# asmekal/ubdvss

Measured on AMD Instinct MI355X. Metric: images/sec (512x512) fwd+CCL, higher is better.
Workload: dtype f32; 1 GPU; configs[1]: batch=32 512x512x3 fp32 forward + CCL postprocess per GPU (stripe-textured rectangle images, random-init weights); batch_per_gpu=32, parallelism=replicas x1, no collective

## Files before the change

ubdvss_amd/csrc/api.hip:

```cpp
#include <stdarg.h>
#include <stddef.h>
#include <stdlib.h>
#include <string.h>
#include <thread>
#include "common.h"

static thread_local char g_err[512] = "";

void ubd_set_error(const char *fmt, ...)
{
    va_list ap;
    va_start(ap, fmt);
    vsnprintf(g_err, sizeof(g_err), fmt, ap);
    va_end(ap);
}

extern "C" const char *ubd_last_error(void) { return g_err; }
extern "C" int ubd_abi_version(void) { return UBD_ABI_VERSION; }
#ifndef UBD_BUILD_ID
#define UBD_BUILD_ID "unknown"
#endif
extern "C" int ubd_host_memcpy_mt(void *dst, const void *src, size_t n, int threads)
{
    if (threads < 1) threads = 1;
// ... 18 lines not shown
    memcpy(dst, src, done_to);
    for (int t = 0; t < started; ++t) th[t].join();
    return 0;
}
extern "C" const char *ubd_build_id(void) { return UBD_BUILD_ID; }

#ifdef UBD_STAMPS
static struct { const char *kernel; ubd_stamp_buf buf; int sel0, sel1; } g_stamps[] = {
    {"stem23"}, {"stem123"}, {"wino"}, {"wino6"}, {"sep123_16"}, {"dilconv16s"}, {"sepb16"}, {"sep_bwd"}, {"dil_wgrad16"}, {"postprocess"}, {"loss"},
};
extern "C" int ubd_debug_set_stamps(const char *kernel, void *buf, size_t capacity_words, int sel0, int sel1)
{
    for (auto &e : g_stamps)
        if (kernel && strcmp(kernel, e.kernel) == 0) {
            e.buf = {(unsigned long long *)buf, buf ? capacity_words : 0};
            e.sel0 = sel0; e.sel1 = sel1;
            return 0;
        }
    UBD_REQUIRE(false, "ubd_debug_set_stamps: no kernel family named %s", kernel ? kernel : "(null)");
}
ubd_stamp_buf ubd_stamps_for(const char *kernel, int sel0, int sel1)
{
    for (const auto &e : g_stamps)
        if (strcmp(kernel, e.kernel) == 0) return e.sel0 == sel0 && e.sel1 == sel1 ? e.buf : ubd_stamp_buf{nullptr, 0};
    return {nullptr, 0};
}
#endif

static const char ANY[] = "", NUMBER[] = "#";
struct env_switch { const char *name; size_t field; const char *value; int set; };
#define SW(name, field, value, set) {name, offsetof(ubd_handle, field), value, set}
static const env_switch ENV_SWITCHES[] = {
    SW("UBD_DILCONV", use_wino, "direct", 0), SW("UBD_DILCONV", wino_x6, "direct", 0), SW("UBD_DILCONV", wino_x6, "wino32", 0),
    SW("UBD_WINO6_LAYOUT", wino6_natural, "natural", 1),
    SW("UBD_STEM", fuse_stem, "fused", UBD_STEM_FUSED23), SW("UBD_STEM", fuse_force, "fused", 1),
    SW("UBD_STEM", fuse_stem, "fused123", UBD_STEM_FUSED123), SW("UBD_STEM", fuse_force, "fused123", 1),
    SW("UBD_STEM", fuse_stem, "unfused", UBD_STEM_SEPARATE),
    SW("UBD_TEST_NUM_CUS", num_cus, NUMBER, 0),
    SW("UBD_DILBWD", split_dilbwd, "split", 1), SW("UBD_DILBWD", no_pair_dilbwd, "pair8", 1),
    SW("UBD_SEPBWD", split_sepbwd32, "split", 1),
    SW("UBD_STEM16", split_stem16, "split", 1), SW("UBD_STEM16", split_stem16, "fused12", 2),
    SW("UBD_PP_GLOBAL", pp_global, ANY, 1), SW("UBD_PP_SPLIT", pp_split, ANY, 1), SW("UBD_PP_POISON", pp_poison, ANY, 1),
    SW("UBD_PP_SERIAL_TAIL", pp_serial_tail, ANY, 1), SW("UBD_PP_THREADS_512", pp_threads_512, ANY, 1),
    SW("UBD_HEADBWD", split_headbwd, "split", 1),
    SW("UBD_SEPB16_X", sepb_x_regs, "regs", 1),
    SW("UBD_REDUCE", chain_reduce, "batched", 0),
    SW("UBD_LOSS", loss_chain, "chain", 1),
    SW("UBD_DILCONV16", direct_dil16, "direct", 1),
};
#undef SW

extern "C" int ubd_create(const ubd_config *cfg, ubd_handle **out)
{
    UBD_REQUIRE(cfg && out, "ubd_create: null argument");
    UBD_REQUIRE(cfg->c_in == 1 || cfg->c_in == 3, "ubd_create: c_in must be 1 (grey) or 3, got %d", cfg->c_in);
    UBD_REQUIRE(cfg->n_classes >= 0 && cfg->n_classes <= UBD_MAX_CLASSES, "ubd_create: n_classes %d out of range [0,%d]", cfg->n_classes, UBD_MAX_CLASSES);
    UBD_REQUIRE(cfg->dtype == UBD_F32 || cfg->dtype == UBD_BF16 || cfg->dtype == UBD_F16, "ubd_create: bad dtype %d", cfg->dtype);
    int ndev = 0;
    hipError_t e = hipGetDeviceCount(&ndev);
    UBD_REQUIRE(e == hipSuccess && ndev > 0, "ubd_create: no HIP device visible (%s); this library has no CPU fallback", hipGetErrorString(e));
    int dev = 0;
    UBD_CHECK_HIP(hipGetDevice(&dev));
    hipDeviceProp_t prop;
    UBD_CHECK_HIP(hipGetDeviceProperties(&prop, dev));
    UBD_REQUIRE(strncmp(prop.gcnArchName, "gfx950", 6) == 0, "ubd_create: device arch %s is not gfx950; this library is built for MI355X only", prop.gcnArchName);

// ... 45 lines not shown
```

ubdvss_amd/csrc/common.h:

```cpp
#pragma once
#include <hip/hip_runtime.h>
#include <stdint.h>
#include <stdio.h>
#include <string.h>
#include <type_traits>
#include "../../include/ubd.h"
#include "stem_plan.h"
#include "stamps.h"

#define UBD_C 24
#define UBD_NUM_DIL 6

struct ubd_comm;
struct ubd_handle {
    ubd_config cfg;
    ubd_comm *comm;
    int k_out;
    size_t off_sep_dw[3], off_sep_pw[3], off_sep_b[3];
    size_t off_dil_k[UBD_NUM_DIL], off_dil_b[UBD_NUM_DIL];
    size_t off_head_k, off_head_b;
    size_t n_params;
    int num_cus;
    int pp_lds_attr_set;
    int stem_cold_tail;
    int fuse_force;
    int split_headbwd;
    int no_pair_dilbwd;
    int split_dilbwd;
    int split_stem16;
    int pp_global, pp_split, pp_poison, pp_serial_tail, pp_threads_512;
    int sepb_x_regs;
    int split_sepbwd32;
    int chain_reduce;
    int direct_dil16;
    int fuse_stem;
    int use_wino;
    int loss_chain;
    int wino_x6;
    int wino6_natural;
};

static const int UBD_DILATIONS[UBD_NUM_DIL] = {1, 2, 4, 8, 16, 1};

#if defined(__HIPCC__)
__device__ __forceinline__ int ubd_xcd_tile(int L, int total)
{
    return (total & 7) == 0 ? (L & 7) * (total >> 3) + (L >> 3) : L;
}
#endif

#if defined(__HIPCC__)
__device__ __forceinline__ void ubd_glds16_at(const void *gsrc, unsigned lds_dst)
{
    unsigned keep;
    asm volatile("s_mov_b32 %0, m0\n\ts_mov_b32 m0, %2\n\ts_nop 0\n\tglobal_load_lds_dwordx4 %1, off\n\ts_mov_b32 m0, %0"
                 : "=&s"(keep) : "v"(gsrc), "s"(lds_dst) : "memory");
}
__device__ __forceinline__ void ubd_glds16_sbase(const void *base_uniform, unsigned voff, unsigned lds_dst)
{
    unsigned keep;
    asm volatile("s_mov_b32 %0, m0\n\ts_mov_b32 m0, %3\n\ts_nop 0\n\tglobal_load_lds_dwordx4 %1, %2\n\ts_mov_b32 m0, %0"
                 : "=&s"(keep) : "v"(voff), "s"(base_uniform), "s"(lds_dst) : "memory");
}
__device__ __forceinline__ void ubd_blds16(__amdgpu_buffer_rsrc_t rsrc, unsigned voff, unsigned lds_dst)
{
    unsigned keep;
    asm volatile("s_mov_b32 %0, m0\n\ts_mov_b32 m0, %3\n\ts_nop 0\n\tbuffer_load_dwordx4 %1, %2, 0 offen lds\n\ts_mov_b32 m0, %0"
                 : "=&s"(keep) : "v"(voff), "s"(rsrc), "s"(lds_dst) : "memory");
}
__device__ __forceinline__ void ubd_blds4(__amdgpu_buffer_rsrc_t rsrc, unsigned voff, unsigned lds_dst)
{
// ... 64 lines not shown
                          hipGetErrorString(_e));                                        \
            return 1;                                                                    \
        }                                                                                \
    } while (0)

#define UBD_REQUIRE(cond, ...)                                                           \
    do {                                                                                 \
        if (!(cond)) {                                                                   \
            ubd_set_error(__VA_ARGS__);                                                  \
            return 2;                                                                    \
        }                                                                                \
    } while (0)

static inline size_t ubd_align_up(size_t v, size_t a) { return (v + a - 1) / a * a; }

static inline bool ubd_pixels_by_lds_dma(bool f32_in, float sub, float div, int H, int W, int c_in, size_t limit, const void *x)
{
    return f32_in && sub == 0.f && div == 1.f && (size_t)H * W * c_in * 4 < limit && ((uintptr_t)x & 15) == 0;
}
static inline bool ubd_head_in_epilogue(const ubd_handle *h) { return h->k_out == 1 && h->off_head_b == h->off_head_k + UBD_C; }
template <int V> using ubd_int = std::integral_constant<int, V>;
template <typename F> static inline void ubd_dispatch_bool(bool b, F f) { if (b) f(std::true_type{}); else f(std::false_type{}); }
template <typename F> static inline void ubd_dispatch_input(int c_in, bool u8, F f)
{
    if (c_in == 1) { if (u8) f(ubd_int<1>{}, ubd_int<1>{}); else f(ubd_int<1>{}, ubd_int<0>{}); }
    else { if (u8) f(ubd_int<3>{}, ubd_int<1>{}); else f(ubd_int<3>{}, ubd_int<0>{}); }
}

#define UBD_DIL_FRAG_FLOATS (9 * 6 * 2 * 64)
#define UBD_SEP_FRAG_FLOATS (6 * 2 * 64)
#define UBD_SEP_DW_FLOATS (9 * 6 * 64)
#define UBD_WINO_FRAG_FLOATS (16 * 6 * 64 * 2)
#define UBD_FWD_DIRECT_FLOATS (3 * (UBD_SEP_FRAG_FLOATS + UBD_SEP_DW_FLOATS) + UBD_NUM_DIL * UBD_DIL_FRAG_FLOATS)
#define UBD_WINO6_FRAG_U32 (16 * 2 * 3 * 64 * 4)
#define UBD_FWD_WINO6_OFF (UBD_FWD_DIRECT_FLOATS + UBD_NUM_DIL * UBD_WINO_FRAG_FLOATS)
#define UBD_FWD_FRAG_FLOATS (UBD_FWD_WINO6_OFF + UBD_NUM_DIL * UBD_WINO6_FRAG_U32)

struct ubd_fwd_layout {
    size_t off_tickets;
    size_t off_wfrag;
    size_t off_a1, off_a2;
    size_t off_b[2];
    size_t off_acts[7];
    size_t total;
};

bool ubd_comm_fused(const ubd_handle *h);
bool ubd_comm_global_loss(const ubd_handle *h);
int ubd_comm_rank(const ubd_handle *h);
enum { UBD_RED_F64 = 0, UBD_RED_I32 = 1, UBD_RED_U32 = 2 };
int ubd_comm_allreduce_raw(ubd_handle *h, void *buf, size_t count, int kind, hipStream_t st);
int ubd_comm_allgather_u32(ubd_handle *h, const unsigned *send_one, unsigned *recv_world, hipStream_t st);
extern "C" int ubd_comm_world(const ubd_handle *h);
int ubd_comm_begin_tail(ubd_handle *h, float *grads, hipStream_t st);
int ubd_comm_finish(ubd_handle *h, float *grads, hipStream_t st);
void ubd_fwd_layout_compute(const ubd_handle *h, int n, int H, int W, int training, ubd_fwd_layout *L);
struct pp_lds_args;
int ubd_forward_impl(ubd_handle *h, const float *params, const void *images, int in_dtype, int preprocessing,
                     int n, int H, int W, float *logits, char *ws, const ubd_fwd_layout &L, hipStream_t st, bool inference = false,
                     const pp_lds_args *pp_job = nullptr);
int ubd_pp_fill_job(ubd_handle *hd, const float *logits, int n, int map_h, int map_w, float logit_threshold, int scale, float min_area,
                    int32_t *binary_map, int32_t *quads, int32_t *classes, int32_t *counts, int cap, void *workspace,
                    size_t workspace_bytes, int threads, pp_lds_args *job);
void ubd_launch_dilconv(const ubd_handle *h, int epi, const float *frag, const float *aux, int dilation,
                        const float *in, float *out, int n, int H4, int W4, hipStream_t st);
int ubd_grid_for(long waves_needed, int num_cus, int waves_per_block, int blocks_per_cu);
int ubd_loss_impl(const float *logits, int k_out, const int32_t *y_true, long npix, float *loss, float *dlogits,
                  char *ws, hipStream_t st, ubd_handle *h = nullptr, bool prezeroed = false);
size_t ubd_loss_zero_bytes(void);
// ... 23 lines not shown
```

ubdvss_amd/csrc/forward.hip:

```cpp
#include "common.h"

typedef float f32x4 __attribute__((ext_vector_type(4)));
typedef float f32x2 __attribute__((ext_vector_type(2)));
typedef unsigned int u32x4 __attribute__((ext_vector_type(4)));
typedef unsigned int u32x2 __attribute__((ext_vector_type(2)));

#include "pack.h"
__global__ void pack_weights_kernel(const float *__restrict__ params, float *__restrict__ wfrag, pack_args a)
{
    pack_weights_body(params, wfrag, a, (int)(blockIdx.x * blockDim.x + threadIdx.x), (int)(gridDim.x * blockDim.x));
}

__device__ __forceinline__ void store_tile_relu(float *__restrict__ y, size_t row_base_elems, int x0, int ow,
                                                int lane, f32x4 acc0, f32x4 acc1, float b0, float b1)
{
    const int co = lane & 15, q = lane >> 4;
    const unsigned long long rp = (unsigned long long)(y + (row_base_elems + (size_t)x0) * UBD_C);
    const unsigned rlo = (unsigned)__builtin_amdgcn_readfirstlane((int)(unsigned)rp);
    const unsigned rhi = (unsigned)__builtin_amdgcn_readfirstlane((int)(unsigned)(rp >> 32));
    float *rowp = (float *)(((unsigned long long)rhi << 32) | rlo);
    int npx = ow - x0 < 16 ? ow - x0 : 16;
    npx = npx < 0 ? 0 : npx;
    const unsigned bytes = (unsigned)__builtin_amdgcn_readfirstlane(npx * UBD_C * 4);
    __amdgpu_buffer_rsrc_t rs = __builtin_amdgcn_make_buffer_rsrc((void *)rowp, 0, (int)bytes, 0x00020000);
// ... 537 lines not shown
void ubd_launch_pack_direct(const ubd_handle *h, const float *params, float *wfrag, hipStream_t st)
{
    pack_args pa;
    for (int s = 0; s < 3; ++s) { pa.off_sep_dw[s] = h->off_sep_dw[s]; pa.off_sep_pw[s] = h->off_sep_pw[s]; }
    for (int k = 0; k < UBD_NUM_DIL; ++k) pa.off_dil_k[k] = h->off_dil_k[k];
    pa.c_in = h->cfg.c_in;
    hipLaunchKernelGGL(pack_weights_kernel, dim3(64), dim3(256), 0, st, params, wfrag, pa);
}

static void launch_pack(const ubd_handle *h, const float *params, float *wfrag, hipStream_t st)
{
    ubd_launch_pack_direct(h, params, wfrag, st);
    if (h->use_wino) ubd_launch_pack_wino(h, params, wfrag + UBD_FWD_DIRECT_FLOATS, 0, st);
    if (h->wino_x6) ubd_launch_pack_wino6(h, params, (unsigned *)(wfrag + UBD_FWD_WINO6_OFF), st);
}

void ubd_launch_dilconv(const ubd_handle *h, int epi, const float *frag, const float *aux, int dilation,
                        const float *in, float *out, int n, int H4, int W4, hipStream_t st)
{
    const unsigned in_bytes = (unsigned)((size_t)n * H4 * W4 * UBD_C * 4);
    const long tiles = (long)n * H4 * ((W4 + 15) / 16);
    int grid = ubd_grid_for(tiles, h->num_cus, 4, 2);
    grid = (grid + 7) / 8 * 8;
    if (epi == 0)
        hipLaunchKernelGGL(dilconv_f32_kernel<0>, dim3(grid), dim3(256), 0, st, in, out, frag, aux, n, H4, W4, dilation, in_bytes);
    else
        hipLaunchKernelGGL(dilconv_f32_kernel<1>, dim3(grid), dim3(256), 0, st, in, out, frag, aux, n, H4, W4, dilation, in_bytes);
}

static void launch_dil(const ubd_handle *h, const float *params, const float *wfrag, int k, const float *in, float *out,
                       int n, int H4, int W4, hipStream_t st, int lay_in = 1, int lay_out = 1)
{
    if (h->wino_x6) {
        ubd_launch_dilconv_wino6(h, 0, (const unsigned *)(wfrag + UBD_FWD_WINO6_OFF) + (size_t)k * UBD_WINO6_FRAG_U32, params + h->off_dil_b[k],
                                 UBD_DILATIONS[k], in, out, n, H4, W4, st, nullptr, lay_in, lay_out);
        return;
    }
    if (h->use_wino) {
        ubd_launch_dilconv_wino(h, 0, wfrag + UBD_FWD_DIRECT_FLOATS + (size_t)k * UBD_WINO_FRAG_FLOATS, params + h->off_dil_b[k], UBD_F32,
                                UBD_DILATIONS[k], in, out, n, H4, W4, st);
        return;
    }
    const int per_sep = UBD_SEP_FRAG_FLOATS + UBD_SEP_DW_FLOATS;
    const float *dfrag = wfrag + 3 * per_sep;
    ubd_launch_dilconv(h, 0, dfrag + (size_t)k * UBD_DIL_FRAG_FLOATS, params + h->off_dil_b[k], UBD_DILATIONS[k], in, out, n, H4, W4, st);
}

extern "C" int ubd_pack_weights(ubd_handle *h, const float *params, void *workspace, size_t workspace_bytes, void *stream)
{
    UBD_REQUIRE(h && params && workspace, "ubd_pack_weights: null argument");
    if (h->cfg.dtype != UBD_F32) return ubd_pack16_workspace(h, params, (char *)workspace, workspace_bytes, (hipStream_t)stream);
    ubd_fwd_layout L;
    ubd_fwd_layout_compute(h, 1, 4, 4, 0, &L);
    UBD_REQUIRE(workspace_bytes >= L.off_a1, "ubd_pack_weights: workspace too small");
    launch_pack(h, params, (float *)((char *)workspace + L.off_wfrag), (hipStream_t)stream);
    UBD_CHECK_HIP(hipMemsetAsync((char *)workspace + L.off_tickets, 0, 256, (hipStream_t)stream));
    UBD_CHECK_HIP(hipGetLastError());
    return 0;
}

extern "C" int ubd_dilated_layer(ubd_handle *h, const float *params, int layer, const void *in, void *out, int n,
                                 int map_h, int map_w, const void *workspace, void *stream)
{
    UBD_REQUIRE(h && params && in && out && workspace, "ubd_dilated_layer: null argument");
    UBD_REQUIRE(layer >= 0 && layer < UBD_NUM_DIL, "ubd_dilated_layer: layer %d out of range", layer);
    UBD_REQUIRE(h->cfg.dtype == UBD_F32, "ubd_dilated_layer: only UBD_F32 in this build");
    UBD_REQUIRE((size_t)n * map_h * map_w * UBD_C * 4 <= (1ull << 30), "ubd_dilated_layer: tensor too large (activation bytes must not exceed 2^30)");
// ... 76 lines not shown
    static_assert(UBD_STEM_STRIP_ROWS == s23_cfg::TH3, "stem_plan.h counts the strips the stem kernels walk");
    const ubd_stem_plan plan = plan_stem_of(h, n, H, W, inference, pp_job ? pp_job->n : -1);
    UBD_REQUIRE(!plan.job_without_strips, "ubd_forward: a postprocess job needs the fused stem kernel (internal error)");
    const bool one_kernel = plan.form == UBD_STEM_FORM_STRIPS || plan.form == UBD_STEM_FORM_COLD;
    static const int phase_lay[UBD_NUM_DIL + 1] = {2, 4, 1, 1, 1, 2, 1};
    const bool phase_major = h->wino_x6 && !h->wino6_natural && one_kernel;
    const int a3_l2p = phase_major ? 1 : 0;
    int *ticket = (int *)(ws + L.off_tickets);
    if (plan.form == UBD_STEM_FORM_COLD)
        launch_stem123<true>(h, params, images, u8, cur, sf0, sf1, sf2, n, H, W, sc, sh, plan.strips * (W4 <= 16 ? 1 : 1 + (W4 - 16 + 14) / 15),
                             ticket, nullptr, a3_l2p, 0, st);
    else if (plan.form == UBD_STEM_FORM_STRIPS)
        launch_stem123<false>(h, params, images, u8, cur, sf0, sf1, sf2, n, H, W, sc, sh, plan.strips, ticket, pp_job, a3_l2p, plan.tail_rows, st);
    else if (h->cfg.c_in == 1)
        launch_sep<1, 2>(h, images, u8, a1, sf0, params + h->off_sep_b[0], n, H, W, H2, W2, pad_s2, sc, sh, st);
    else
        launch_sep<3, 2>(h, images, u8, a1, sf0, params + h->off_sep_b[0], n, H, W, H2, W2, pad_s2, sc, sh, st);
    if (plan.form == UBD_STEM_FORM_L1_STEM23) {
        const int grid = plan.strips < h->num_cus ? (int)plan.strips : h->num_cus;
        ubd_dispatch_bool(pad_s2 != 0, [&](auto pad) {
            hipLaunchKernelGGL(stem23_kernel<decltype(pad)::value>, dim3(grid), dim3(s23_cfg::NT), 0, st, a1, cur, sf1, params + h->off_sep_b[1], sf2,
                               params + h->off_sep_b[2], n, H2, W2, H4, W4, pad_s2 UBD_STAMP_ARG("stem23"));
        });
    } else if (plan.form == UBD_STEM_FORM_SEPARATE) {
        launch_sep<UBD_C, 1>(h, a1, 0, a2, sf1, params + h->off_sep_b[1], n, H2, W2, H2, W2, 1, 0.f, 1.f, st);
        launch_sep<UBD_C, 2>(h, a2, 0, cur, sf2, params + h->off_sep_b[2], n, H2, W2, H4, W4, pad_s2, 0.f, 1.f, st);
    }

    const bool fuse_head = inference && h->use_wino && ubd_head_in_epilogue(h);
    for (int k = 0; k < UBD_NUM_DIL; ++k) {
        float *nxt = (float *)(ws + L.off_acts[k + 1]);
        if (fuse_head && k == UBD_NUM_DIL - 1) {
            if (h->wino_x6)
                ubd_launch_dilconv_wino6(h, 2, (const unsigned *)(wfrag + UBD_FWD_WINO6_OFF) + (size_t)k * UBD_WINO6_FRAG_U32, params + h->off_dil_b[k],
                                         UBD_DILATIONS[k], cur, logits, n, H4, W4, st, params + h->off_head_k, phase_major ? phase_lay[k] : 1, 1);
            else
                ubd_launch_dilconv_wino(h, 2, wfrag + UBD_FWD_DIRECT_FLOATS + (size_t)k * UBD_WINO_FRAG_FLOATS, params + h->off_dil_b[k], UBD_F32,
                                        UBD_DILATIONS[k], cur, logits, n, H4, W4, st, params + h->off_head_k);
            UBD_CHECK_HIP(hipGetLastError());
            return 0;
        }
        launch_dil(h, params, wfrag, k, cur, nxt, n, H4, W4, st, phase_major ? phase_lay[k] : 1, phase_major ? phase_lay[k + 1] : 1);
        cur = nxt;
    }
    const long npix = (long)n * H4 * W4;
    int hgrid = (int)((npix + 255) / 256);
    if (hgrid > h->num_cus * 8) hgrid = h->num_cus * 8;
    hipLaunchKernelGGL(head_kernel, dim3(hgrid), dim3(256), 0, st, cur, logits, params + h->off_head_k, params + h->off_head_b, npix, h->k_out);
    UBD_CHECK_HIP(hipGetLastError());
    return 0;
}

static int forward_f32(ubd_handle *h, const float *params, const void *images, int in_dtype, int preprocessing, int n, int H, int W, float *logits,
                       void *workspace, size_t workspace_bytes, void *stream, const pp_lds_args *pp_job)
{
    ubd_fwd_layout L;
    ubd_fwd_layout_compute(h, n, H, W, 0, &L);
    UBD_REQUIRE(workspace_bytes >= L.total, "ubd_forward: workspace too small (%zu < %zu)", workspace_bytes, L.total);
    return ubd_forward_impl(h, params, images, in_dtype, preprocessing, n, H, W, logits, (char *)workspace, L, (hipStream_t)stream, true, pp_job);
}

extern "C" int ubd_forward(ubd_handle *h, const float *params, const void *images, int in_dtype, int preprocessing,
                           int n, int height, int width, float *logits, void *workspace, size_t workspace_bytes,
                           void *stream)
{
    UBD_REQUIRE(h && params && images && logits && workspace, "ubd_forward: null argument");
    if (h->cfg.dtype != UBD_F32) {
// ... 29 lines not shown
```

ubdvss_amd/csrc/wino6.hip:

```cpp
#include "common.h"
#include "split3.h"

struct wino6_pack_args { size_t off_dil_k[UBD_NUM_DIL]; };

__global__ void pack_wino6_kernel(const float *__restrict__ params, unsigned *__restrict__ out, wino6_pack_args a)
{
    const float G[4][3] = {{1.f, 0.f, 0.f}, {0.5f, 0.5f, 0.5f}, {0.5f, -0.5f, 0.5f}, {0.f, 0.f, 1.f}};
    const int total = UBD_NUM_DIL * 16 * 2 * 64;
    for (int idx = blockIdx.x * blockDim.x + threadIdx.x; idx < total; idx += gridDim.x * blockDim.x) {
        const int lane = idx & 63, nt = (idx >> 6) & 1, xi = (idx >> 7) & 15, L = idx >> 11;
        const int q = lane >> 4, co = (lane & 15) + 16 * nt;
        const int ta = xi >> 2, tb = xi & 3;
        unsigned p[3][4] = {{0, 0, 0, 0}, {0, 0, 0, 0}, {0, 0, 0, 0}};
        if (co < UBD_C) {
            const float *wk = params + a.off_dil_k[L];
            for (int e = 0; e < 6; ++e) {
                const int ci = e < 4 ? 4 * q + e : 16 + 2 * q + (e - 4);
                float v = 0.f;
                for (int ky = 0; ky < 3; ++ky)
                    for (int kx = 0; kx < 3; ++kx)
                        v += G[ta][ky] * G[tb][kx] * wk[((ky * 3 + kx) * UBD_C + ci) * UBD_C + co];
                unsigned b[3];
                split3_bits(v, b);
                const int sh = (e & 1) ? 0 : 16;
                p[0][e >> 1] |= b[0] >> sh;
                p[1][e >> 1] |= b[1] >> sh;
                p[2][e >> 1] |= b[2] >> sh;
            }
        }
        unsigned *o = out + ((size_t)(idx >> 6) * 3 * 64 + lane) * 4;
#pragma unroll
        for (int pc = 0; pc < 3; ++pc)
            *(u32x4 *)(o + pc * 64 * 4) = (u32x4){p[pc][0], p[pc][1], p[pc][2], p[pc][3]};
    }
}

void ubd_launch_pack_wino6(const ubd_handle *h, const float *params, unsigned *out, hipStream_t st)
{
    wino6_pack_args a;
    for (int k = 0; k < UBD_NUM_DIL; ++k) a.off_dil_k[k] = h->off_dil_k[k];
    hipLaunchKernelGGL(pack_wino6_kernel, dim3(48), dim3(256), 0, st, params, out, a);
}


#define WSTAMP(cond, k) UBD_STAMP(cond, ((size_t)blockIdx.x * W6_WAVES + wave_in_block) * 8 + (k))

#ifndef W6_WAVES
#define W6_WAVES 8
#endif
struct w6samples {
    f32x4 v4[4][4];
    f32x2 v2[4][4];
};
struct w6geom {
    int n, h, w, d, log2d;
    unsigned in_bytes;
    unsigned groups_x, half_rows, total;
    unsigned magic_gx, magic_hr;
    int wpb;
    int phase;
    int l2po;
};
struct w6addr {
    unsigned row[4];
    unsigned lrow[2];
    unsigned c4[4];
    unsigned c2[4];
    unsigned oc[2];
};

template <int EPI, bool LAY>
__global__ __launch_bounds__(64 * W6_WAVES) void dilconv_wino6_kernel(const float *__restrict__ x, float *__restrict__ y,
                                                                     const unsigned *__restrict__ ufrag,
                                                                     const float *__restrict__ bias, w6geom G, const float *__restrict__ head UBD_STAMP_PARAM)
{
    __shared__ __attribute__((aligned(16))) unsigned s_u[UBD_WINO6_FRAG_U32];
    const int lane = threadIdx.x & 63;
    const int i = lane & 15, q = lane >> 4;
    const int h = G.h, w = G.w, d = G.d, log2d = G.log2d, dm1 = G.d - 1;
    const f32x4 bA = *(const f32x4 *)(bias + 4 * q);
    const f32x4 bB = q < 2 ? *(const f32x4 *)(bias + 16 + 4 * q) : (f32x4){0.f, 0.f, 0.f, 0.f};
    f32x4 hA = {0.f, 0.f, 0.f, 0.f}, hB = {0.f, 0.f, 0.f, 0.f};
    float hbias = 0.f;
    if constexpr (EPI == 2) {
        hA = *(const f32x4 *)(head + 4 * q);
        if (q < 2) hB = *(const f32x4 *)(head + 16 + 4 * q);
        hbias = head[UBD_C];
    }
    const int xcd = blockIdx.x & 7;
    const int nblk_x = (gridDim.x + 7 - xcd) >> 3;
    const int chunk = (int)((G.total + 7) >> 3);
    const int g_begin = xcd * chunk;
    const int g_end = (g_begin + chunk < (int)G.total) ? g_begin + chunk : (int)G.total;
    const int stride = nblk_x * G.wpb;

    __amdgpu_buffer_rsrc_t rsrc = __builtin_amdgcn_make_buffer_rsrc((void *)x, 0, (int)G.in_bytes, 0x00020000);
    __amdgpu_buffer_rsrc_t yrsrc = __builtin_amdgcn_make_buffer_rsrc((void *)y, 0, (int)(EPI == 2 ? G.in_bytes / UBD_C : G.in_bytes), 0x00020000);

    const int wave_in_block = __builtin_amdgcn_readfirstlane((int)(threadIdx.x >> 6));
    int g = g_begin + (int)(blockIdx.x >> 3) * G.wpb + wave_in_block;
    const int g_last = g_end - 1;
    const unsigned BIG = 0x40000000u;
    const unsigned lane4 = 16u * q, lane2 = 64u + 8u * q;

    auto set_addr = [&](w6addr &A, int gg) {
        const unsigned rs = G.groups_x == 1u ? (unsigned)gg : __umulhi((unsigned)gg, G.magic_gx);
        const unsigned gx = (unsigned)gg - rs * G.groups_x;
        const unsigned img = G.half_rows == 1u ? rs : __umulhi(rs, G.magic_hr);
        const unsigned s = rs - img * G.half_rows;
        const int y0 = (int)(((s >> log2d) << (log2d + 1)) + (s & (unsigned)dm1));
        const unsigned img_row = img * (unsigned)h;
#pragma unroll
        for (int a = 0; a < 4; ++a) {
            const int iy = y0 + (a - 1) * d;
            const bool ok = iy >= 0 && iy < h;
            A.row[a] = ok ? (img_row + (unsigned)iy) * (unsigned)w * (unsigned)(UBD_C * 4) : BIG;
            if (EPI == 2 && (a == 1 || a == 2)) A.lrow[a - 1] = ok ? (img_row + (unsigned)iy) * (unsigned)w * 4u : BIG;
        }
        const int ph = (int)(gx & (unsigned)dm1);
        const int tk = (int)((gx >> log2d) << 4) + i;
        const bool phase = LAY && G.phase;
// ... 9 lines not shown
            const int sb = phase ? rb * wq + (rb < wr ? rb : wr) + (r >> l2p) : (b - 1) * d;
            const unsigned cb = (unsigned)(tl + sb) * (unsigned)(UBD_C * 4);
            A.c4[b] = ok ? cb + lane4 : BIG;
            A.c2[b] = ok ? cb + lane2 : BIG;
        }
        if constexpr (LAY) {
#pragma unroll
            for (int c = 0; c < 2; ++c) {
                const int ox = xj + c * d;
                const int r = ox & ((1 << G.l2po) - 1);
                const int wrp = w & ((1 << G.l2po) - 1);
                const int pos = r * (w >> G.l2po) + (r < wrp ? r : wrp) + (ox >> G.l2po);
                A.oc[c] = ox < w ? (unsigned)pos * (unsigned)(UBD_C * 4) + lane4 : BIG;
            }
        } else {
            A.oc[0] = A.c4[1]; A.oc[1] = A.c4[2];
        }
    };
    auto load_row = [&](w6samples &D, const w6addr &A, int a) {
#pragma unroll
        for (int b = 0; b < 4; ++b) {
            D.v4[a][b] = __builtin_bit_cast(f32x4, __builtin_amdgcn_raw_buffer_load_b128(rsrc, (int)A.c4[b], (int)A.row[a], 0));
            D.v2[a][b] = __builtin_bit_cast(f32x2, __builtin_amdgcn_raw_buffer_load_b64(rsrc, (int)A.c2[b], (int)A.row[a], 0));
        }
    };

    w6samples D;
    w6addr A, An;
    WSTAMP(true, 0);
    set_addr(A, g < g_last ? g : g_last);
    load_row(D, A, 0);
    load_row(D, A, 2);
    load_row(D, A, 1);
    constexpr int PER_WAVE = UBD_WINO6_FRAG_U32 * 4 / 1024 / W6_WAVES;
    constexpr int EARLY_ROUNDS = 4 * 6 / W6_WAVES;
    static_assert(PER_WAVE - EARLY_ROUNDS == 9, "the counted wait below is written for nine late rounds");
    {
        const unsigned lds_u = ubd_lds_addr(s_u);
#pragma unroll
        for (int k = 0; k < PER_WAVE; ++k) {
            const int piece = k * W6_WAVES + wave_in_block;
            ubd_glds16_sbase((const char *)ufrag + (size_t)piece * 1024, (unsigned)lane * 16u, lds_u + (unsigned)piece * 1024u);
        }
    }
    asm volatile("s_waitcnt vmcnt(9)" ::: "memory");
    __builtin_amdgcn_s_barrier();
    WSTAMP(true, 1);
    if (g >= g_end || wave_in_block >= G.wpb) {
        asm volatile("s_waitcnt vmcnt(0)" ::: "memory");
        __builtin_amdgcn_s_barrier();
        return;
    }
    bool weights_pending = true;
    [[maybe_unused]] int gcount = 0;
    const u32x4 *su4 = (const u32x4 *)s_u + lane;
    for (;;) {
        f32x4 Y[2][2][2];
        f32x4 Z0[2], Z1[2];
        f32x4 V4[4];
        f32x2 V2[4];
        auto make_v = [&](int a) {
            f32x4 T4[4];
            f32x2 T2[4];
#pragma unroll
            for (int b = 0; b < 4; ++b) {
                if (a == 0) { T4[b] = D.v4[0][b] - D.v4[2][b]; T2[b] = D.v2[0][b] - D.v2[2][b]; }
                else if (a == 1) { T4[b] = D.v4[1][b] + D.v4[2][b]; T2[b] = D.v2[1][b] + D.v2[2][b]; }
                else if (a == 2) { T4[b] = D.v4[2][b] - D.v4[1][b]; T2[b] = D.v2[2][b] - D.v2[1][b]; }
                else { T4[b] = D.v4[1][b] - D.v4[3][b]; T2[b] = D.v2[1][b] - D.v2[3][b]; }
            }
            V4[0] = T4[0] - T4[2]; V4[1] = T4[1] + T4[2]; V4[2] = T4[2] - T4[1]; V4[3] = T4[1] - T4[3];
            V2[0] = T2[0] - T2[2]; V2[1] = T2[1] + T2[2]; V2[2] = T2[2] - T2[1]; V2[3] = T2[1] - T2[3];
        };
        auto consume = [&](int a, int b, const f32x4 (&m)[2]) {
#pragma unroll
            for (int nt = 0; nt < 2; ++nt) {
                if (b == 0) Z0[nt] = m[nt];
                else if (b == 1) { Z0[nt] += m[nt]; Z1[nt] = m[nt]; }
                else if (b == 2) { Z0[nt] += m[nt]; Z1[nt] -= m[nt]; }
                else {
                    Z1[nt] -= m[nt];
                    if (a == 0) { Y[0][0][nt] = Z0[nt]; Y[0][1][nt] = Z1[nt]; }
                    else if (a == 1) { Y[0][0][nt] += Z0[nt]; Y[0][1][nt] += Z1[nt]; Y[1][0][nt] = Z0[nt]; Y[1][1][nt] = Z1[nt]; }
                    else if (a == 2) { Y[0][0][nt] += Z0[nt]; Y[0][1][nt] += Z1[nt]; Y[1][0][nt] -= Z0[nt]; Y[1][1][nt] -= Z1[nt]; }
                    else { Y[1][0][nt] -= Z0[nt]; Y[1][1][nt] -= Z1[nt]; }
                }
            }
        };
        make_v(0);
        u32x4 U[2][3];
        u32x4 P1, P2, P3;
        f32x4 r4, t4;
        f32x2 r2, t2;
        auto load_u = [&](int xi) {
#pragma unroll
            for (int nt = 0; nt < 2; ++nt)
#pragma unroll
                for (int pc = 0; pc < 3; ++pc) U[nt][pc] = su4[((xi * 2 + nt) * 3 + pc) * 64];
        };
        load_u(0);
        r4 = resid(V4[0]); t4 = resid(r4); r2 = resid(V2[0]); t2 = resid(r2);
        P1 = pack6(V4[0], V2[0]); P2 = pack6(r4, r2); P3 = pack6(t4, t2);
#pragma unroll
        for (int xi = 0; xi < 16; ++xi) {
            const int a = xi >> 2, b = xi & 3;
            __builtin_amdgcn_sched_barrier(0);
            f32x4 m[2] = {{0.f, 0.f, 0.f, 0.f}, {0.f, 0.f, 0.f, 0.f}};
            m[0] = mfma16(U[0][2], P1, m[0]); m[1] = mfma16(U[1][2], P1, m[1]);
            m[0] = mfma16(U[0][0], P3, m[0]); m[1] = mfma16(U[1][0], P3, m[1]);
            m[0] = mfma16(U[0][1], P2, m[0]); m[1] = mfma16(U[1][1], P2, m[1]);
            m[0] = mfma16(U[0][1], P1, m[0]); m[1] = mfma16(U[1][1], P1, m[1]);
            m[0] = mfma16(U[0][0], P2, m[0]); m[1] = mfma16(U[1][0], P2, m[1]);
            m[0] = mfma16(U[0][0], P1, m[0]); m[1] = mfma16(U[1][0], P1, m[1]);
            if (b < 3) { r4 = resid(V4[b + 1]); t4 = resid(r4); r2 = resid(V2[b + 1]); t2 = resid(r2); }
#pragma unroll
            for (int k = 0; k < 12; ++k) {
                __builtin_amdgcn_sched_group_barrier(0x008, 1, 0);
                __builtin_amdgcn_sched_group_barrier(0x002, 2, 0);
            }
            __builtin_amdgcn_sched_barrier(0);
            if (xi == 3 && weights_pending) {
                asm volatile("s_waitcnt vmcnt(0)" ::: "memory");
                __builtin_amdgcn_s_barrier();
                weights_pending = false;
            }
            if (xi < 15) load_u(xi + 1);
            if (b == 3 && a < 3) {
                make_v(a + 1);
                if (a == 1) load_row(D, A, 3);
                if (a == 2) {
                    const int gn = g + stride;
                    set_addr(An, gn < g_last ? gn : g_last);
                    load_row(D, An, 0);
                    load_row(D, An, 2);
                }
                r4 = resid(V4[0]); t4 = resid(r4); r2 = resid(V2[0]); t2 = resid(r2);
            }
            if (xi < 15) { const int bn = (b + 1) & 3; P1 = pack6(V4[bn], V2[bn]); P2 = pack6(r4, r2); P3 = pack6(t4, t2); }
            consume(a, b, m);
            WSTAMP(gcount == 1 && (xi & 3) == 3, 2 + (xi >> 2));
        }
        load_row(D, An, 1);

        {
#pragma unroll
            for (int rr = 0; rr < 2; ++rr)
#pragma unroll
                for (int c = 0; c < 2; ++c) {
                    f32x4 v0 = Y[rr][c][0] + bA, v1 = Y[rr][c][1] + bB;
#pragma unroll
                    for (int r = 0; r < 4; ++r) { v0[r] = fmaxf(v0[r], 0.f); v1[r] = fmaxf(v1[r], 0.f); }
                    if constexpr (EPI == 2) {
                        float part = 0.f;
#pragma unroll
                        for (int r = 0; r < 4; ++r) part = fmaf(v0[r], hA[r], part);
#pragma unroll
                        for (int r = 0; r < 4; ++r) part = fmaf(v1[r], hB[r], part);
                        part += __shfl_xor(part, 16, 64);
                        part += __shfl_xor(part, 32, 64);
                        const unsigned lcol = (q == 0 && A.oc[c] != BIG) ? A.oc[c] / (unsigned)UBD_C : BIG;
                        __builtin_amdgcn_raw_buffer_store_b32(__builtin_bit_cast(unsigned, part + hbias), yrsrc, (int)(lcol + A.lrow[rr]), 0, 0);
                    } else {
                        const unsigned st1 = (q < 2 && A.oc[c] != BIG) ? A.oc[c] + 64u : BIG;
                        __builtin_amdgcn_raw_buffer_store_b128(__builtin_bit_cast(u32x4, v0), yrsrc, (int)(A.oc[c] + A.row[1 + rr]), 0, 0);
                        __builtin_amdgcn_raw_buffer_store_b128(__builtin_bit_cast(u32x4, v1), yrsrc, (int)(st1 + A.row[1 + rr]), 0, 0);
                    }
                }
        }
        WSTAMP(gcount == 1, 6);
        WSTAMP(gcount == 0, 1);
        ++gcount;
        g += stride;
        if (g >= g_end) break;
        A = An;
    }
    WSTAMP(true, 7);
}

static int ilog2(int v) { int l = 0; while ((1 << l) < v) ++l; return l; }

void ubd_launch_dilconv_wino6(const ubd_handle *h, int epi, const unsigned *frag, const float *bias, int dilation,
                              const float *in, float *out, int n, int H4, int W4, hipStream_t st, const float *head,
                              int lay_in, int lay_out)
{
    const int d = dilation;
    const long half_rows = ((H4 + 2 * d - 1) / (2 * d)) * d, half_cols = ((W4 + 2 * d - 1) / (2 * d)) * d;
    const long groups_x = lay_in == 1 ? (half_cols + 15) / 16 : (long)d * ((half_cols / d + 15) / 16);
    const long groups = (long)n * half_rows * groups_x;
    w6geom G;
    G.n = n; G.h = H4; G.w = W4; G.d = d; G.log2d = ilog2(d);
    G.phase = lay_in != 1; G.l2po = ilog2(lay_out);
    G.in_bytes = (unsigned)((size_t)n * H4 * W4 * UBD_C * 4);
    G.groups_x = (unsigned)groups_x; G.half_rows = (unsigned)half_rows; G.total = (unsigned)groups;
    G.magic_gx = groups_x == 1 ? 0u : (unsigned)(0xFFFFFFFFul / (unsigned long)groups_x + 1ul);
    G.magic_hr = half_rows == 1 ? 0u : (unsigned)(0xFFFFFFFFul / (unsigned long)half_rows + 1ul);
    int wpb = (int)((groups + h->num_cus - 1) / h->num_cus);
    if (wpb < 1) wpb = 1;
    if (wpb > W6_WAVES) wpb = W6_WAVES;
    G.wpb = wpb;
    int grid = ubd_grid_for(groups, h->num_cus, wpb, 1);
    grid = (grid + 7) / 8 * 8;
    const bool lay = lay_in != 1 || lay_out != 1;
    if (epi == 2 && lay)
        hipLaunchKernelGGL((dilconv_wino6_kernel<2, true>), dim3(grid), dim3(64 * W6_WAVES), 0, st, in, out, frag, bias, G, head UBD_STAMP_ARG("wino6"));
    else if (epi == 2)
        hipLaunchKernelGGL((dilconv_wino6_kernel<2, false>), dim3(grid), dim3(64 * W6_WAVES), 0, st, in, out, frag, bias, G, head UBD_STAMP_ARG("wino6"));
    else if (lay)
        hipLaunchKernelGGL((dilconv_wino6_kernel<0, true>), dim3(grid), dim3(64 * W6_WAVES), 0, st, in, out, frag, bias, G, nullptr UBD_STAMP_ARG("wino6"));
    else
        hipLaunchKernelGGL((dilconv_wino6_kernel<0, false>), dim3(grid), dim3(64 * W6_WAVES), 0, st, in, out, frag, bias, G, nullptr UBD_STAMP_ARG("wino6"));
}
```

Baseline: 103,100 images/s.

## Use two-piece scaled f16 split for Winograd-6 MFMA instead of three-piece split

Replaces the default three-piece split (split3) emulation of fp32 in the wino6 dilated-conv kernel with a two-piece f16 hi/lo split, backed by per-tile dynamic scaling of the transformed input and a per-layer scale on the weights. This drops each 6-element product from 9 to 6 MFMAs (hi*hi, hi*lo, lo*hi) and shrinks the weight fragment and its LDS footprint from 3 pieces to 2. In exchange it adds scale computation through permlane swaps and extra multiplies in the output accumulation. Dropping the lo*lo term and relying on f16 range under scaling may lose some accuracy compared with the split3 path.

Result: faster. 110,500 images/s (median of 6 runs) (+7.2%).

```diff
diff --git a/ubdvss_amd/csrc/api.hip b/ubdvss_amd/csrc/api.hip
--- a/ubdvss_amd/csrc/api.hip
+++ b/ubdvss_amd/csrc/api.hip
@@ -74,6 +74,7 @@
 #define SW(name, field, value, set) {name, offsetof(ubd_handle, field), value, set}
 static const env_switch ENV_SWITCHES[] = {
     SW("UBD_DILCONV", use_wino, "direct", 0), SW("UBD_DILCONV", wino_x6, "direct", 0), SW("UBD_DILCONV", wino_x6, "wino32", 0),
+    SW("UBD_DILCONV", wino6_split3, "split3", 1),
     SW("UBD_WINO6_LAYOUT", wino6_natural, "natural", 1),
     SW("UBD_STEM", fuse_stem, "fused", UBD_STEM_FUSED23), SW("UBD_STEM", fuse_force, "fused", 1),
     SW("UBD_STEM", fuse_stem, "fused123", UBD_STEM_FUSED123), SW("UBD_STEM", fuse_force, "fused123", 1),
diff --git a/ubdvss_amd/csrc/common.h b/ubdvss_amd/csrc/common.h
--- a/ubdvss_amd/csrc/common.h
+++ b/ubdvss_amd/csrc/common.h
@@ -37,6 +37,7 @@
     int use_wino;
     int loss_chain;
     int wino_x6;
+    int wino6_split3;
     int wino6_natural;
 };
 
@@ -167,9 +168,11 @@
 #define UBD_SEP_DW_FLOATS (9 * 6 * 64)
 #define UBD_WINO_FRAG_FLOATS (16 * 6 * 64 * 2)
 #define UBD_FWD_DIRECT_FLOATS (3 * (UBD_SEP_FRAG_FLOATS + UBD_SEP_DW_FLOATS) + UBD_NUM_DIL * UBD_DIL_FRAG_FLOATS)
-#define UBD_WINO6_FRAG_U32 (16 * 2 * 3 * 64 * 4)
+#define UBD_WINO6_FRAG_U32 (16 * 2 * 2 * 64 * 4)
+#define UBD_WINO6_FRAG3_U32 (16 * 2 * 3 * 64 * 4)
+#define UBD_WINO6_SLOT_U32 UBD_WINO6_FRAG3_U32
 #define UBD_FWD_WINO6_OFF (UBD_FWD_DIRECT_FLOATS + UBD_NUM_DIL * UBD_WINO_FRAG_FLOATS)
-#define UBD_FWD_FRAG_FLOATS (UBD_FWD_WINO6_OFF + UBD_NUM_DIL * UBD_WINO6_FRAG_U32)
+#define UBD_FWD_FRAG_FLOATS (UBD_FWD_WINO6_OFF + UBD_NUM_DIL * UBD_WINO6_SLOT_U32)
 
 struct ubd_fwd_layout {
     size_t off_tickets;
diff --git a/ubdvss_amd/csrc/forward.hip b/ubdvss_amd/csrc/forward.hip
--- a/ubdvss_amd/csrc/forward.hip
+++ b/ubdvss_amd/csrc/forward.hip
@@ -593,7 +593,7 @@
                        int n, int H4, int W4, hipStream_t st, int lay_in = 1, int lay_out = 1)
 {
     if (h->wino_x6) {
-        ubd_launch_dilconv_wino6(h, 0, (const unsigned *)(wfrag + UBD_FWD_WINO6_OFF) + (size_t)k * UBD_WINO6_FRAG_U32, params + h->off_dil_b[k],
+        ubd_launch_dilconv_wino6(h, 0, (const unsigned *)(wfrag + UBD_FWD_WINO6_OFF) + (size_t)k * UBD_WINO6_SLOT_U32, params + h->off_dil_b[k],
                                  UBD_DILATIONS[k], in, out, n, H4, W4, st, nullptr, lay_in, lay_out);
         return;
     }
@@ -736,7 +736,7 @@
         float *nxt = (float *)(ws + L.off_acts[k + 1]);
         if (fuse_head && k == UBD_NUM_DIL - 1) {
             if (h->wino_x6)
-                ubd_launch_dilconv_wino6(h, 2, (const unsigned *)(wfrag + UBD_FWD_WINO6_OFF) + (size_t)k * UBD_WINO6_FRAG_U32, params + h->off_dil_b[k],
+                ubd_launch_dilconv_wino6(h, 2, (const unsigned *)(wfrag + UBD_FWD_WINO6_OFF) + (size_t)k * UBD_WINO6_SLOT_U32, params + h->off_dil_b[k],
                                          UBD_DILATIONS[k], cur, logits, n, H4, W4, st, params + h->off_head_k, phase_major ? phase_lay[k] : 1, 1);
             else
                 ubd_launch_dilconv_wino(h, 2, wfrag + UBD_FWD_DIRECT_FLOATS + (size_t)k * UBD_WINO_FRAG_FLOATS, params + h->off_dil_b[k], UBD_F32,
diff --git a/ubdvss_amd/csrc/split2h.h b/ubdvss_amd/csrc/split2h.h
--- /dev/null
+++ b/ubdvss_amd/csrc/split2h.h
@@ -0,0 +1,93 @@
+#pragma once
+
+#if defined(__HIPCC__)
+#define SPLIT2H_FN __host__ __device__ __forceinline__
+#else
+#include <cstring>
+#define SPLIT2H_FN inline
+#endif
+
+SPLIT2H_FN unsigned split2h_bits(float v)
+{
+#if defined(__HIPCC__)
+    return __builtin_bit_cast(unsigned, v);
+#else
+    unsigned u; memcpy(&u, &v, 4); return u;
+#endif
+}
+SPLIT2H_FN float split2h_float(unsigned u)
+{
+#if defined(__HIPCC__)
+    return __builtin_bit_cast(float, u);
+#else
+    float v; memcpy(&v, &u, 4); return v;
+#endif
+}
+
+#define SPLIT2H_SAMPLE_TOP 13
+#define SPLIT2H_SAMPLE_LO 40
+#define SPLIT2H_WEIGHT_TOP 12
+#define SPLIT2H_WEIGHT_LO 90
+
+SPLIT2H_FN void split2h_scale(unsigned maxbits, int top, int lo, unsigned &s_bits, unsigned &inv_bits)
+{
+    int e = (int)(maxbits >> 23);
+    e = e < lo ? lo : (e > 254 ? 254 : e);
+    const bool zero = maxbits == 0u;
+    s_bits = zero ? 0x3f800000u : (unsigned)(254 + top - e) << 23;
+    inv_bits = zero ? 0x3f800000u : (unsigned)(e - top) << 23;
+}
+
+SPLIT2H_FN float split2h_round_f16(float x)
+{
+    const unsigned u = split2h_bits(x), sign = u & 0x80000000u, a = u & 0x7fffffffu;
+    if (a >= 0x7f800000u) return x;
+    if (a < 0x38800000u) {
+        const float m = split2h_float(a);
+        const float r = (m + 0.5f) - 0.5f;
+        return split2h_float(split2h_bits(r) | sign);
+    }
+    unsigned r = a + 0xfffu + ((a >> 13) & 1u);
+    r &= 0xffffe000u;
+    if (r >= 0x47800000u) r = 0x7f800000u;
+    return split2h_float(r | sign);
+}
+
+SPLIT2H_FN void split2h_pieces(float xs, float &h1, float &h2)
+{
+    h1 = split2h_round_f16(xs);
+    h2 = split2h_round_f16(xs - h1);
+}
+
+#if defined(__HIPCC__)
+typedef float f32x4 __attribute__((ext_vector_type(4)));
+typedef float f32x2 __attribute__((ext_vector_type(2)));
+typedef unsigned int u32x4 __attribute__((ext_vector_type(4)));
+typedef _Float16 f16x2 __attribute__((ext_vector_type(2)));
+typedef _Float16 f16x8 __attribute__((ext_vector_type(8)));
+
+__device__ __forceinline__ unsigned split2h_f16_bits(float h) { return (unsigned)__builtin_bit_cast(unsigned short, (_Float16)h); }
+
+__device__ __forceinline__ void split2h_pair(float a, float b, unsigned &p1, unsigned &p2)
+{
+    const f32x2 v = {a, b};
+    const f16x2 h1 = __builtin_convertvector(v, f16x2);
+    const f32x2 r = v - __builtin_convertvector(h1, f32x2);
+    const f16x2 h2 = __builtin_convertvector(r, f16x2);
+    p1 = __builtin_bit_cast(unsigned, h1);
+    p2 = __builtin_bit_cast(unsigned, h2);
+}
+__device__ __forceinline__ void split2h_6(f32x4 a, f32x2 b, u32x4 &P1, u32x4 &P2)
+{
+    unsigned p1[3], p2[3];
+    split2h_pair(a[0], a[1], p1[0], p2[0]);
+    split2h_pair(a[2], a[3], p1[1], p2[1]);
+    split2h_pair(b[0], b[1], p1[2], p2[2]);
+    P1 = (u32x4){p1[0], p1[1], p1[2], 0u};
+    P2 = (u32x4){p2[0], p2[1], p2[2], 0u};
+}
+__device__ __forceinline__ f32x4 mfma16h(u32x4 a, u32x4 b, f32x4 c)
+{
+    return __builtin_amdgcn_mfma_f32_16x16x32_f16(__builtin_bit_cast(f16x8, a), __builtin_bit_cast(f16x8, b), c, 0, 0, 0);
+}
+#endif
diff --git a/ubdvss_amd/csrc/wino6.hip b/ubdvss_amd/csrc/wino6.hip
--- a/ubdvss_amd/csrc/wino6.hip
+++ b/ubdvss_amd/csrc/wino6.hip
@@ -1,5 +1,6 @@
 #include "common.h"
 #include "split3.h"
+#include "split2h.h"
 
 struct wino6_pack_args { size_t off_dil_k[UBD_NUM_DIL]; };
 
@@ -35,11 +36,65 @@
     }
 }
 
+#define W6_PACK_BLOCKS 4
+__device__ __forceinline__ float wino6_u(const float *wk, int ta, int tb, int ci, int co)
+{
+    const float G[4][3] = {{1.f, 0.f, 0.f}, {0.5f, 0.5f, 0.5f}, {0.5f, -0.5f, 0.5f}, {0.f, 0.f, 1.f}};
+    float v = 0.f;
+    for (int ky = 0; ky < 3; ++ky)
+        for (int kx = 0; kx < 3; ++kx)
+            v += G[ta][ky] * G[tb][kx] * wk[((ky * 3 + kx) * UBD_C + ci) * UBD_C + co];
+    return v;
+}
+__global__ __launch_bounds__(1024) void pack_wino6h_kernel(const float *__restrict__ params, unsigned *__restrict__ out, wino6_pack_args a)
+{
+    __shared__ unsigned s_max;
+    const int L = blockIdx.x / W6_PACK_BLOCKS, part = blockIdx.x % W6_PACK_BLOCKS;
+    const float *wk = params + a.off_dil_k[L];
+    if (threadIdx.x == 0) s_max = 0u;
+    __syncthreads();
+    unsigned mx = 0u;
+    for (int j = threadIdx.x; j < 16 * UBD_C * UBD_C; j += blockDim.x) {
+        const int co = j % UBD_C, ci = (j / UBD_C) % UBD_C, xi = j / (UBD_C * UBD_C);
+        const unsigned b = split2h_bits(wino6_u(wk, xi >> 2, xi & 3, ci, co)) & 0x7fffffffu;
+        mx = b > mx ? b : mx;
+    }
+    atomicMax(&s_max, mx);
+    __syncthreads();
+    unsigned t_bits, inv_bits;
+    split2h_scale(s_max, SPLIT2H_WEIGHT_TOP, SPLIT2H_WEIGHT_LO, t_bits, inv_bits);
+    const float t = split2h_float(t_bits);
+    unsigned *slot = out + (size_t)L * UBD_WINO6_SLOT_U32;
+    if (part == 0 && threadIdx.x == 0) slot[UBD_WINO6_FRAG_U32] = inv_bits;
+    const int per_block = 16 * 2 * 64 / W6_PACK_BLOCKS;
+    for (int k = threadIdx.x; k < per_block; k += blockDim.x) {
+        const int idx = part * per_block + k;
+        const int lane = idx & 63, nt = (idx >> 6) & 1, xi = idx >> 7;
+        const int q = lane >> 4, co = (lane & 15) + 16 * nt;
+        unsigned p[2][4] = {{0, 0, 0, 0}, {0, 0, 0, 0}};
+        if (co < UBD_C) {
+            for (int e = 0; e < 6; ++e) {
+                const int ci = e < 4 ? 4 * q + e : 16 + 2 * q + (e - 4);
+                float g1, g2;
+                split2h_pieces(wino6_u(wk, xi >> 2, xi & 3, ci, co) * t, g1, g2);
+                const int sh = (e & 1) ? 16 : 0;
+                p[0][e >> 1] |= split2h_f16_bits(g1) << sh;
+                p[1][e >> 1] |= split2h_f16_bits(g2) << sh;
+            }
+        }
+        unsigned *o = slot + ((size_t)(idx >> 6) * 2 * 64 + lane) * 4;
+#pragma unroll
+        for (int pc = 0; pc < 2; ++pc)
+            *(u32x4 *)(o + pc * 64 * 4) = (u32x4){p[pc][0], p[pc][1], p[pc][2], p[pc][3]};
+    }
+}
+
 void ubd_launch_pack_wino6(const ubd_handle *h, const float *params, unsigned *out, hipStream_t st)
 {
     wino6_pack_args a;
     for (int k = 0; k < UBD_NUM_DIL; ++k) a.off_dil_k[k] = h->off_dil_k[k];
-    hipLaunchKernelGGL(pack_wino6_kernel, dim3(48), dim3(256), 0, st, params, out, a);
+    if (h->wino6_split3) hipLaunchKernelGGL(pack_wino6_kernel, dim3(48), dim3(256), 0, st, params, out, a);
+    else hipLaunchKernelGGL(pack_wino6h_kernel, dim3(UBD_NUM_DIL * W6_PACK_BLOCKS), dim3(1024), 0, st, params, out, a);
 }
 
 
@@ -69,12 +124,14 @@
     unsigned oc[2];
 };
 
-template <int EPI, bool LAY>
+template <int EPI, bool LAY, bool F16 = true>
 __global__ __launch_bounds__(64 * W6_WAVES) void dilconv_wino6_kernel(const float *__restrict__ x, float *__restrict__ y,
                                                                      const unsigned *__restrict__ ufrag,
                                                                      const float *__restrict__ bias, w6geom G, const float *__restrict__ head UBD_STAMP_PARAM)
 {
-    __shared__ __attribute__((aligned(16))) unsigned s_u[UBD_WINO6_FRAG_U32];
+    constexpr int NPC = F16 ? 2 : 3;
+    constexpr int FRAG_U32 = F16 ? UBD_WINO6_FRAG_U32 : UBD_WINO6_FRAG3_U32;
+    __shared__ __attribute__((aligned(16))) unsigned s_u[FRAG_U32];
     const int lane = threadIdx.x & 63;
     const int i = lane & 15, q = lane >> 4;
     const int h = G.h, w = G.w, d = G.d, log2d = G.log2d, dm1 = G.d - 1;
@@ -87,6 +144,8 @@
         if (q < 2) hB = *(const f32x4 *)(head + 16 + 4 * q);
         hbias = head[UBD_C];
     }
+    [[maybe_unused]] float inv_t = 1.f;
+    if constexpr (F16) inv_t = __builtin_bit_cast(float, ufrag[UBD_WINO6_FRAG_U32]);
     const int xcd = blockIdx.x & 7;
     const int nblk_x = (gridDim.x + 7 - xcd) >> 3;
     const int chunk = (int)((G.total + 7) >> 3);
@@ -162,9 +221,9 @@
     load_row(D, A, 0);
     load_row(D, A, 2);
     load_row(D, A, 1);
-    constexpr int PER_WAVE = UBD_WINO6_FRAG_U32 * 4 / 1024 / W6_WAVES;
-    constexpr int EARLY_ROUNDS = 4 * 6 / W6_WAVES;
-    static_assert(PER_WAVE - EARLY_ROUNDS == 9, "the counted wait below is written for nine late rounds");
+    constexpr int PER_WAVE = FRAG_U32 * 4 / 1024 / W6_WAVES;
+    constexpr int EARLY_ROUNDS = 4 * 2 * NPC / W6_WAVES;
+    static_assert(PER_WAVE - EARLY_ROUNDS == (F16 ? 6 : 9), "the counted wait below is written for six (nine) late rounds");
     {
         const unsigned lds_u = ubd_lds_addr(s_u);
 #pragma unroll
@@ -173,7 +232,8 @@
             ubd_glds16_sbase((const char *)ufrag + (size_t)piece * 1024, (unsigned)lane * 16u, lds_u + (unsigned)piece * 1024u);
         }
     }
-    asm volatile("s_waitcnt vmcnt(9)" ::: "memory");
+    if constexpr (F16) asm volatile("s_waitcnt vmcnt(6)" ::: "memory");
+    else asm volatile("s_waitcnt vmcnt(9)" ::: "memory");
     __builtin_amdgcn_s_barrier();
     WSTAMP(true, 1);
     if (g >= g_end || wave_in_block >= G.wpb) {
@@ -189,6 +249,7 @@
         f32x4 Z0[2], Z1[2];
         f32x4 V4[4];
         f32x2 V2[4];
+        [[maybe_unused]] float inv_s[4];
         auto make_v = [&](int a) {
             f32x4 T4[4];
             f32x2 T2[4];
@@ -199,6 +260,26 @@
                 else if (a == 2) { T4[b] = D.v4[2][b] - D.v4[1][b]; T2[b] = D.v2[2][b] - D.v2[1][b]; }
                 else { T4[b] = D.v4[1][b] - D.v4[3][b]; T2[b] = D.v2[1][b] - D.v2[3][b]; }
             }
+            if constexpr (F16) {
+                float mx = 0.f;
+#pragma unroll
+                for (int b = 0; b < 4; ++b) {
+                    mx = fmaxf(fmaxf(fabsf(T4[b][0]), fabsf(T4[b][1])), mx);
+                    mx = fmaxf(fmaxf(fabsf(T4[b][2]), fabsf(T4[b][3])), mx);
+                    mx = fmaxf(fmaxf(fabsf(T2[b][0]), fabsf(T2[b][1])), mx);
+                }
+                unsigned mb = __builtin_bit_cast(unsigned, mx);
+                const u32x2 h16 = __builtin_amdgcn_permlane16_swap(mb, mb, false, false);
+                mb = h16[0] > h16[1] ? h16[0] : h16[1];
+                const u32x2 h32 = __builtin_amdgcn_permlane32_swap(mb, mb, false, false);
+                mb = h32[0] > h32[1] ? h32[0] : h32[1];
+                unsigned s_bits, inv_bits;
+                split2h_scale(mb, SPLIT2H_SAMPLE_TOP, SPLIT2H_SAMPLE_LO, s_bits, inv_bits);
+                const float s = __builtin_bit_cast(float, s_bits);
+                inv_s[a] = __builtin_bit_cast(float, inv_bits) * inv_t;
+#pragma unroll
+                for (int b = 0; b < 4; ++b) { T4[b] *= s; T2[b] *= s; }
+            }
             V4[0] = T4[0] - T4[2]; V4[1] = T4[1] + T4[2]; V4[2] = T4[2] - T4[1]; V4[3] = T4[1] - T4[3];
             V2[0] = T2[0] - T2[2]; V2[1] = T2[1] + T2[2]; V2[2] = T2[2] - T2[1]; V2[3] = T2[1] - T2[3];
         };
@@ -208,7 +289,19 @@
                 if (b == 0) Z0[nt] = m[nt];
                 else if (b == 1) { Z0[nt] += m[nt]; Z1[nt] = m[nt]; }
                 else if (b == 2) { Z0[nt] += m[nt]; Z1[nt] -= m[nt]; }
-                else {
+                else if constexpr (F16) {
+                    Z1[nt] -= m[nt];
+                    const float iv = inv_s[a];
+                    f32x4 &y00 = Y[0][0][nt], &y01 = Y[0][1][nt], &y10 = Y[1][0][nt], &y11 = Y[1][1][nt];
+#pragma unroll
+                    for (int r = 0; r < 4; ++r) {
+                        const float z0 = Z0[nt][r], z1 = Z1[nt][r];
+                        if (a == 0) { y00[r] = z0 * iv; y01[r] = z1 * iv; }
+                        else if (a == 1) { y00[r] = fmaf(z0, iv, y00[r]); y01[r] = fmaf(z1, iv, y01[r]); y10[r] = z0 * iv; y11[r] = z1 * iv; }
+                        else if (a == 2) { y00[r] = fmaf(z0, iv, y00[r]); y01[r] = fmaf(z1, iv, y01[r]); y10[r] = fmaf(-z0, iv, y10[r]); y11[r] = fmaf(-z1, iv, y11[r]); }
+                        else { y10[r] = fmaf(-z0, iv, y10[r]); y11[r] = fmaf(-z1, iv, y11[r]); }
+                    }
+                } else {
                     Z1[nt] -= m[nt];
                     if (a == 0) { Y[0][0][nt] = Z0[nt]; Y[0][1][nt] = Z1[nt]; }
                     else if (a == 1) { Y[0][0][nt] += Z0[nt]; Y[0][1][nt] += Z1[nt]; Y[1][0][nt] = Z0[nt]; Y[1][1][nt] = Z1[nt]; }
@@ -218,6 +311,54 @@
             }
         };
         make_v(0);
+        if constexpr (F16) {
+        u32x4 U[2][2];
+        u32x4 P1, P2, N1, N2;
+        auto load_u = [&](int xi) {
+#pragma unroll
+            for (int nt = 0; nt < 2; ++nt)
+#pragma unroll
+                for (int pc = 0; pc < 2; ++pc) U[nt][pc] = su4[((xi * 2 + nt) * 2 + pc) * 64];
+        };
+        load_u(0);
+        split2h_6(V4[0], V2[0], P1, P2);
+#pragma unroll
+        for (int xi = 0; xi < 16; ++xi) {
+            const int a = xi >> 2, b = xi & 3;
+            __builtin_amdgcn_sched_barrier(0);
+            f32x4 m[2] = {{0.f, 0.f, 0.f, 0.f}, {0.f, 0.f, 0.f, 0.f}};
+            m[0] = mfma16h(U[0][0], P2, m[0]); m[1] = mfma16h(U[1][0], P2, m[1]);
+            m[0] = mfma16h(U[0][1], P1, m[0]); m[1] = mfma16h(U[1][1], P1, m[1]);
+            m[0] = mfma16h(U[0][0], P1, m[0]); m[1] = mfma16h(U[1][0], P1, m[1]);
+            if (b < 3) split2h_6(V4[b + 1], V2[b + 1], N1, N2);
+#pragma unroll
+            for (int k = 0; k < 6; ++k) {
+                __builtin_amdgcn_sched_group_barrier(0x008, 1, 0);
+                __builtin_amdgcn_sched_group_barrier(0x002, 3, 0);
+            }
+            __builtin_amdgcn_sched_barrier(0);
+            if (xi == 3 && weights_pending) {
+                asm volatile("s_waitcnt vmcnt(0)" ::: "memory");
+                __builtin_amdgcn_s_barrier();
+                weights_pending = false;
+            }
+            if (xi < 15) load_u(xi + 1);
+            if (b == 3 && a < 3) {
+                make_v(a + 1);
+                if (a == 1) load_row(D, A, 3);
+                if (a == 2) {
+                    const int gn = g + stride;
+                    set_addr(An, gn < g_last ? gn : g_last);
+                    load_row(D, An, 0);
+                    load_row(D, An, 2);
+                }
+                split2h_6(V4[0], V2[0], N1, N2);
+            }
+            if (xi < 15) { P1 = N1; P2 = N2; }
+            consume(a, b, m);
+            WSTAMP(gcount == 1 && (xi & 3) == 3, 2 + (xi >> 2));
+        }
+        } else {
         u32x4 U[2][3];
         u32x4 P1, P2, P3;
         f32x4 r4, t4;
@@ -269,6 +410,7 @@
             if (xi < 15) { const int bn = (b + 1) & 3; P1 = pack6(V4[bn], V2[bn]); P2 = pack6(r4, r2); P3 = pack6(t4, t2); }
             consume(a, b, m);
             WSTAMP(gcount == 1 && (xi & 3) == 3, 2 + (xi >> 2));
+        }
         }
         load_row(D, An, 1);
 
@@ -331,12 +473,15 @@
     int grid = ubd_grid_for(groups, h->num_cus, wpb, 1);
     grid = (grid + 7) / 8 * 8;
     const bool lay = lay_in != 1 || lay_out != 1;
-    if (epi == 2 && lay)
-        hipLaunchKernelGGL((dilconv_wino6_kernel<2, true>), dim3(grid), dim3(64 * W6_WAVES), 0, st, in, out, frag, bias, G, head UBD_STAMP_ARG("wino6"));
-    else if (epi == 2)
-        hipLaunchKernelGGL((dilconv_wino6_kernel<2, false>), dim3(grid), dim3(64 * W6_WAVES), 0, st, in, out, frag, bias, G, head UBD_STAMP_ARG("wino6"));
-    else if (lay)
-        hipLaunchKernelGGL((dilconv_wino6_kernel<0, true>), dim3(grid), dim3(64 * W6_WAVES), 0, st, in, out, frag, bias, G, nullptr UBD_STAMP_ARG("wino6"));
-    else
-        hipLaunchKernelGGL((dilconv_wino6_kernel<0, false>), dim3(grid), dim3(64 * W6_WAVES), 0, st, in, out, frag, bias, G, nullptr UBD_STAMP_ARG("wino6"));
-}
+    ubd_dispatch_bool(h->wino6_split3 == 0, [&](auto f16_tag) {
+        constexpr bool F16 = decltype(f16_tag)::value;
+        if (epi == 2 && lay)
+            hipLaunchKernelGGL((dilconv_wino6_kernel<2, true, F16>), dim3(grid), dim3(64 * W6_WAVES), 0, st, in, out, frag, bias, G, head UBD_STAMP_ARG("wino6"));
+        else if (epi == 2)
+            hipLaunchKernelGGL((dilconv_wino6_kernel<2, false, F16>), dim3(grid), dim3(64 * W6_WAVES), 0, st, in, out, frag, bias, G, head UBD_STAMP_ARG("wino6"));
+        else if (lay)
+            hipLaunchKernelGGL((dilconv_wino6_kernel<0, true, F16>), dim3(grid), dim3(64 * W6_WAVES), 0, st, in, out, frag, bias, G, nullptr UBD_STAMP_ARG("wino6"));
+        else
+            hipLaunchKernelGGL((dilconv_wino6_kernel<0, false, F16>), dim3(grid), dim3(64 * W6_WAVES), 0, st, in, out, frag, bias, G, nullptr UBD_STAMP_ARG("wino6"));
+    });
+}
```
